# ReallyNecessarySherbert/VoxelHex

Hardware: AMD Instinct MI355X
Metric: primary Mrays/s at 3840×2160 on 1024³ brick tree; achieved HBM GB/s % (higher is better)
Workload: dtype f32; 1 GPU; primary rays 3840x2160, 1024^3 procedural scene S (lattice+cube), brick_dim 4, glass camera; workload_key=primary 3840x2160 S1 1024^3 bd4 ranks1, tree_size=1024, brick_dim=4, width=3840, height=2160, scene=1, parallelism=single GPU, tree_nodes=187246, tree_bricks=11796480

## Files before the change

### voxelhex_amd/csrc/ctx.hpp

```cpp
#pragma once
#include <hip/hip_runtime.h>

#include <condition_variable>
#include <cstdint>
#include <memory>
#include <mutex>
#include <string>
#include <vector>

#include "../../include/vhx.h"

struct DevBuf {
    void *ptr = nullptr;
    uint64_t bytes = 0;
};

struct TreeStore {
    int device = 0;
    bool uploaded = false;
    vhx_tree_desc desc{};
    DevBuf raw[7];
    DevBuf hdr, brick_occ;
    DevBuf child_rec;
    bool child_rec_stale = false;
// ... 67 lines not shown
    DevBuf upd;
    DevBuf query;
    hipStream_t upd_stream = nullptr;
    struct BuildScratch {
        DevBuf occ, rank, first, part, table, ctl, grid, simp;
    } build;
    struct EditScratch {
        DevBuf oldn, aft, need, rank, nmask, first, ctl;
    } edit;
    struct CompactScratch {
        DevBuf new_of, old_of, nmask, nrank, bmask, bfirst, bnew, bsrc, ctl;
    } compact;
    bool prepass = false, in_prepass = false;
    bool shadow_on = false;
    float shadow_light[3] = {0.f, 0.f, 0.f};
    bool keep_ev0 = false;
    uint32_t shadow_budget = 0;
    bool tail_on = false;
    uint32_t tail_min = 512, tail_cap = 4096, tail_rpw = 4, tail_prio = 0;
    DevBuf tail_list[2], tail_mask;
    uint32_t tail_cur = 0, tail_w = 0, tail_h = 0;
    bool tail_valid = false;
    uint32_t *tail_rec = nullptr;
    hipStream_t tail_stream = nullptr;
    hipEvent_t tail_fork = nullptr, tail_join = nullptr;
    float prepass_margin = 0.0f;
    DevBuf prepass_depth;
    struct Sched {
        uint32_t budgets[VHX_MAX_BUDGETS];
        uint32_t npass;
        uint32_t sparse[VHX_MAX_BUDGETS];
        uint32_t queue_waves_per_cu;
        uint32_t qorder;
        uint32_t qsort;
        uint32_t queue_waves0_per_cu;
        uint32_t shadow_budgets[VHX_MAX_BUDGETS];
        uint32_t shadow_npass;
    };
    bool adaptive = true;
    Sched sched_busy = {{32u, 128u, 768u}, 4u, {12u}, 3u, VHX_QORDER_BUSY, VHX_QSORT_BUSY, 4u, {24u, 72u, 216u, 648u}, 5u};
    Sched sched_idle = {{64u}, 2u, {0u}, 8u, VHX_QORDER_IDLE, VHX_QSORT_IDLE, 32u, {64u}, 2u};
    int last_sched = -1;
    uint32_t budgets[VHX_MAX_BUDGETS] = {32u, 128u, 768u};
    uint32_t npass = 4;
    uint32_t rpw[VHX_MAX_BUDGETS + 1] = {64u, 64u, 64u, 64u, 64u, 64u, 64u};
    uint32_t tw = 1024;
    uint32_t scan_multi = 8;
    bool p0lists = true;
    bool resume = true;
    bool qstate = false;
    bool tile_lists = true;
    bool frame_interleave = true;
    bool skyblocks = true;
    DevBuf sky;
    uint32_t save_from = 0;
    uint32_t xcd_group = 16;
    uint32_t qblock = 256;
    uint32_t queue_blocks = 2048;
    uint32_t queue_waves = 1024;
    uint32_t cus = 256;
    uint32_t queue_waves0 = 8192;
    uint32_t queue_waves0_force = 0;
    uint32_t queue_waves_mid = 0;
    uint32_t qxcd = 16;
    bool qxcd_all = false;
    uint32_t qorder = VHX_QORDER_BUSY;
    uint32_t last_fb_w = 0, last_fb_h = 0;
    uint32_t sparse[VHX_MAX_BUDGETS] = {12u};
    uint32_t qsort = 0;
    int qsort_force = -1;
    uint32_t qsort_passes = 0xFEu;
    uint32_t qsort_blocks = 2048u;
};

#define VHX_HIP(ctx, call)                                                                                         \
    do {                                                                                                           \
        hipError_t e_ = (call);                                                                                    \
        if (e_ != hipSuccess) {                                                                                    \
            (ctx)->err = std::string(#call) + ": " + hipGetErrorString(e_);                                        \
            return VHX_E_HIP;                                                                                      \
        }                                                                                                          \
    } while (0)

#define VHX_STREAM(ctx)                                                                                            \
    do {                                                                                                           \
        if (!(ctx)->stream) {                                                                                      \
            if (!(ctx)->own_stream) VHX_HIP(ctx, hipStreamCreateWithFlags(&(ctx)->own_stream, hipStreamNonBlocking)); \
            (ctx)->stream = (ctx)->own_stream;                                                                     \
        }                                                                                                          \
    } while (0)

static inline int fail(vhx_ctx *ctx, int code, const char *msg) {
    if (ctx) ctx->err = msg;
    return code;
}
static inline int fail(vhx_ctx *ctx, int code, const std::string &msg) { return fail(ctx, code, msg.c_str()); }

namespace vhx {
int ensure(vhx_ctx *c, DevBuf &b, uint64_t bytes);
uint64_t elem_size(int id);
uint64_t elem_count(const vhx_tree_desc &d, int id);
int alloc_tree(vhx_ctx *c, const vhx_tree_desc *t);
int grow_tree(vhx_ctx *c, const vhx_tree_desc *t);
int finish_upload(vhx_ctx *c);
struct FreshTree {
    DevBuf raw[7], hdr, brick_occ, child_rec;
};
// ... 53 lines not shown
```

### voxelhex_amd/csrc/vhx_ctx.hip

```cpp
#include <hip/hip_runtime.h>

#include <algorithm>
#include <cmath>
#include <cstdio>
#include <cstdlib>
#include <cstring>
#include <string>
#include <vector>

#include "../../include/vhx.h"
#include "ctx.hpp"

using namespace vhx;

__global__ void __launch_bounds__(256) k_untile_planes(const uint32_t *__restrict__ gathered, uint32_t planes,
                                                       uint32_t ranks, uint32_t tiles_per_rank, uint32_t T,
                                                       uint32_t tiles_x, uint32_t ntiles, uint32_t width,
                                                       uint32_t height, uint32_t *__restrict__ fb0,
                                                       uint32_t *__restrict__ fb1) {
    const uint64_t i = (uint64_t)blockIdx.x * blockDim.x + threadIdx.x;
    const uint64_t per_plane = (uint64_t)tiles_per_rank * T * T, per_rank = per_plane * planes;
    if (i >= per_rank * ranks) return;
    const uint32_t r = (uint32_t)(i / per_rank);
    const uint64_t w = i - (uint64_t)r * per_rank;
// ... 128 lines not shown
    if (hipGetDeviceCount(&n) != hipSuccess || n == 0) return VHX_E_NO_DEVICE;
    if (hip_device < 0 || hip_device >= n) return VHX_E_INVALID_ARG;
    vhx_ctx *c = new vhx_ctx();
    c->device = hip_device;
    c->tree = std::make_shared<TreeStore>();
    c->tree->device = hip_device;
    register_user(c);
    auto bail = [&](const char *what, hipError_t e) {
        fprintf(stderr, "vhx_create: %s: %s\n", what, hipGetErrorString(e));
        delete c;
        return VHX_E_HIP;
    };
    hipError_t e;
    if ((e = hipSetDevice(hip_device)) != hipSuccess) return bail("hipSetDevice", e);
    {
        hipDeviceProp_t prop;
        if (hipGetDeviceProperties(&prop, hip_device) == hipSuccess && prop.multiProcessorCount > 0) {
            c->cus = (uint32_t)prop.multiProcessorCount;
            c->queue_blocks = c->cus * 8u;
            c->queue_waves = c->sched_busy.queue_waves_per_cu * c->cus;
        }
    }
    if ((e = hipEventCreate(&c->ev0)) != hipSuccess) return bail("hipEventCreate", e);
    if ((e = hipEventCreate(&c->ev1)) != hipSuccess) return bail("hipEventCreate", e);
    *out = c;
    return VHX_OK;
}

int vhx_create_shared(const vhx_ctx *owner, vhx_ctx **out) {
    if (!owner || !out) return VHX_E_INVALID_ARG;
    *out = nullptr;
    vhx_ctx *c = nullptr;
    int rc = vhx_create(owner->device, &c);
    if (rc) return rc;
    c->tree = owner->tree;
    register_user(c);
    c->shared = true;
    copy_sched(c, owner);
    *out = c;
    return VHX_OK;
}

void vhx_destroy(vhx_ctx *c) {
    if (!c) return;
    (void)hipSetDevice(c->device);
    if (c->stream) (void)hipStreamSynchronize(c->stream);
    unregister_user(c);
    c->tree.reset();
    if (c->use_ev) (void)hipEventDestroy(c->use_ev);
    for (DevBuf *b : {&c->scratch, &c->rays, &c->queue[0], &c->queue[1], &c->qctl, &c->tmp, &c->counts, &c->offsets,
                      &c->flags, &c->qargs, &c->state, &c->stateq, &c->upd, &c->prepass_depth, &c->batch_args, &c->scan_part,
                      &c->shadow_args, &c->tail_list[0], &c->tail_list[1], &c->tail_mask, &c->build.occ, &c->build.rank,
                      &c->build.first, &c->build.part, &c->build.table, &c->build.ctl, &c->build.grid,
                      &c->build.simp, &c->sky, &c->query, &c->edit.oldn, &c->edit.aft, &c->edit.need,
                      &c->edit.rank, &c->edit.nmask, &c->edit.first, &c->edit.ctl, &c->compact.new_of,
                      &c->compact.old_of, &c->compact.nmask, &c->compact.nrank, &c->compact.bmask,
                      &c->compact.bfirst, &c->compact.bnew, &c->compact.bsrc, &c->compact.ctl})
        if (b->ptr) (void)hipFree(b->ptr);
    if (c->tail_stream) {
        (void)hipStreamSynchronize(c->tail_stream);
        (void)hipStreamDestroy(c->tail_stream);
    }
    if (c->tail_fork) (void)hipEventDestroy(c->tail_fork);
    if (c->tail_join) (void)hipEventDestroy(c->tail_join);
    std::vector<vhx_ctx::Pinned *> pins = {&c->pinned[0], &c->pinned[1]};
    for (auto &P : c->batch_pinned) pins.push_back(&P);
    for (auto &P : c->shadow_pinned) pins.push_back(&P);
    for (auto *P : pins) {
        if (P->ptr) (void)hipHostFree(P->ptr);
        if (P->done) (void)hipEventDestroy(P->done);
    }
    if (c->ev0) (void)hipEventDestroy(c->ev0);
    if (c->ev1) (void)hipEventDestroy(c->ev1);
    if (c->own_stream) (void)hipStreamDestroy(c->own_stream);
    delete c;
}

static bool parse_u32_list(const std::string &v, uint32_t *out, uint32_t cap, uint32_t &n) {
    n = 0;
    const char *q = v.c_str();
    if (!*q) return true;
    for (;;) {
        char *end = nullptr;
        const unsigned long x = strtoul(q, &end, 10);
        if (end == q || n >= cap || x > 0xFFFFFFFFul) return false;
        out[n++] = (uint32_t)x;
        if (*end == '\0') return true;
        if (*end != ',') return false;
        q = end + 1;
    }
}
static bool parse_u32(const std::string &v, uint32_t &out) {
    uint32_t n = 0, x[1];
    if (!parse_u32_list(v, x, 1, n) || n != 1) return false;
    out = x[0];
    return true;
}
static int apply_tuning(vhx_ctx *c, const std::string &key, const std::string &val) {
    uint32_t x = 0, n = 0, l[VHX_MAX_BUDGETS + 1];
    auto bad = [&]() { return fail(c, VHX_E_INVALID_ARG, ("vhx_set_tuning: bad value for " + key).c_str()); };
    if (key == "budgets") {
        if (!parse_u32_list(val, l, VHX_MAX_BUDGETS, n)) return bad();
        if (n == 1 && l[0] == 0) n = 0;
        return vhx_set_pass_budgets(c, l, n);
    } else if (key == "adaptive") {
        if (!parse_u32(val, x) || x > 1) return bad();
        return vhx_set_adaptive_schedule(c, (int)x);
// ... 304 lines not shown
```

### voxelhex_amd/csrc/vhx_device.hip

```cpp
#include <hip/hip_runtime.h>

#include <algorithm>
#include <cmath>
#include <cstdio>
#include <cstdlib>
#include <cstring>
#include <string>
#include <vector>

#include "../../include/vhx.h"
#include "trace.hpp"
#define VHX_SKY_FN __host__ __device__
#include "skyblock.hpp"
static_assert(VHX_RAY_GLASS == 1u, "skyblock.hpp spells the glass model's number out (it includes no header)");

using namespace vhx;

#include "ctx.hpp"

struct CamD {
    uint32_t model, width, height;
    float ox, oy, oz;
    float blx, bly, blz, rx, ry, rz, ux, uy, uz, pw, ph;
    float m[16];
};

struct OutD {
    uint32_t *value, *cell, *voxel, *rgba, *bytes;
    float *impact, *normal, *depth;
    uint32_t *shadowed;
};

__device__ __forceinline__ uint32_t shade(const DevTree &t, const HitOut &h) {
    if (!h.hit) return 128u | (128u << 8) | (128u << 16) | (255u << 24);
    const uint32_t ci = h.value & 0xFFFFu;
    if (ci == 0xFFFFu || ci >= t.color_count) return 255u << 24;
    const uint32_t c = t.color[ci];
    const F3d L = vnorm(mk(0.0f, -1.0f, 1.0f));
    const float dot = (h.nx * L.x + h.ny * L.y) + h.nz * L.z;
    const float s = 1.0f - (dot / 2.0f + 0.5f);
    const uint32_t r = ras_u8((float)(c & 0xFFu) * s), g = ras_u8((float)((c >> 8) & 0xFFu) * s),
                   b = ras_u8((float)((c >> 16) & 0xFFu) * s);
    return r | (g << 8) | (b << 16) | (255u << 24);
}

__device__ __forceinline__ void store(const DevTree &t, const OutD &o, uint64_t i, F3d org, const HitOut &h) {
    if (o.value) o.value[i] = h.hit ? h.value : VHX_EMPTY;
    if (o.cell) o.cell[i] = h.hit ? h.cell : VHX_EMPTY;
    if (o.voxel) {
        o.voxel[3 * i] = h.hit ? h.vx : VHX_EMPTY;
        o.voxel[3 * i + 1] = h.hit ? h.vy : VHX_EMPTY;
        o.voxel[3 * i + 2] = h.hit ? h.vz : VHX_EMPTY;
    }
    if (o.impact) {
        o.impact[3 * i] = h.hit ? h.ix : 0.0f;
        o.impact[3 * i + 1] = h.hit ? h.iy : 0.0f;
        o.impact[3 * i + 2] = h.hit ? h.iz : 0.0f;
    }
    if (o.normal) {
        o.normal[3 * i] = h.hit ? h.nx : 0.0f;
        o.normal[3 * i + 1] = h.hit ? h.ny : 0.0f;
        o.normal[3 * i + 2] = h.hit ? h.nz : 0.0f;
    }
    if (o.depth) o.depth[i] = h.hit ? vlen(vsub(mk(h.ix, h.iy, h.iz), org)) : __builtin_huge_valf();
    if (o.rgba) o.rgba[i] = shade(t, h);
    if (o.bytes) o.bytes[i] = h.bytes;
}

__device__ __forceinline__ void primary_ray(const CamD &c, uint32_t px, uint32_t py, F3d &o, F3d &d) {
    const uint32_t x = px, y = c.height - 1u - py;
    o = mk(c.ox, c.oy, c.oz);
    if (c.model == VHX_RAY_GLASS) {
        const F3d gp = vadd(vadd(mk(c.blx, c.bly, c.blz), vmul(vmul(mk(c.rx, c.ry, c.rz), (float)x), c.pw)),
                            vmul(vmul(mk(c.ux, c.uy, c.uz), (float)y), c.ph));
        d = vnorm(vsub(gp, o));
    } else {
        const float nx = ((float)x + 0.5f) / (float)c.width * 2.0f - 1.0f;
        const float ny = ((float)y + 0.5f) / (float)c.height * 2.0f - 1.0f;
        float nr[4], fr[4];
#pragma unroll
        for (int k = 0; k < 4; ++k) {
            nr[k] = ((c.m[k] * nx + c.m[4 + k] * ny) + c.m[8 + k] * -1.0f) + c.m[12 + k] * 1.0f;
            fr[k] = ((c.m[k] * nx + c.m[4 + k] * ny) + c.m[8 + k] * 1.0f) + c.m[12 + k] * 1.0f;
        }
        const F3d np = mk(nr[0] / nr[3], nr[1] / nr[3], nr[2] / nr[3]);
        const F3d fp = mk(fr[0] / fr[3], fr[1] / fr[3], fr[2] / fr[3]);
        const F3d dd = vsub(fp, np);
        const float rcp = 1.0f / __builtin_sqrtf((dd.x * dd.x + dd.y * dd.y) + dd.z * dd.z);
        d = vmul(dd, rcp);
    }
}

__device__ __forceinline__ bool glass_clear_miss(const CamD &c, uint32_t px, uint32_t py, float tsize) {
    if (c.model != VHX_RAY_GLASS) return false;
    const uint32_t x = px, y = c.height - 1u - py;
    const F3d o = mk(c.ox, c.oy, c.oz);
    const F3d gp = vadd(vadd(mk(c.blx, c.bly, c.blz), vmul(vmul(mk(c.rx, c.ry, c.rz), (float)x), c.pw)),
                        vmul(vmul(mk(c.ux, c.uy, c.uz), (float)y), c.ph));
    const F3d v = vsub(gp, o);
    const float vk[3] = {v.x, v.y, v.z}, ok[3] = {o.x, o.y, o.z};
    float tmin = -__builtin_huge_valf(), tmax = __builtin_huge_valf();
    bool safe = true;
#pragma unroll
    for (int k = 0; k < 3; ++k) {
        safe = safe && __builtin_fabsf(vk[k]) > 1e-20f;
        const float r = __builtin_amdgcn_rcpf(vk[k]);
        const float t1 = (0.0f - ok[k]) * r, t2 = (tsize - ok[k]) * r;
        tmin = __builtin_fmaxf(tmin, __builtin_fminf(t1, t2));
        tmax = __builtin_fminf(tmax, __builtin_fmaxf(t1, t2));
    }
    if (!safe || !__builtin_isfinite(tmin) || !__builtin_isfinite(tmax)) return false;
    const float m = 1e-5f * __builtin_fmaxf(__builtin_fabsf(tmin), __builtin_fabsf(tmax));
    return tmax < -m || tmin - tmax > m;
}

__global__ void __launch_bounds__(256) k_classify_sky(const CamD *__restrict__ cams, uint32_t nfr, uint32_t blocks_x,
                                                      uint32_t blocks_y, uint32_t tree_size,
                                                      uint8_t *__restrict__ mask) {
    const uint32_t nb = blocks_x * blocks_y;
    const uint32_t i = blockIdx.x * 256u + threadIdx.x;
    if (i >= nfr * nb) return;
    const uint32_t f = i / nb, b = i - f * nb, by = b / blocks_x, bx = b - by * blocks_x;
    const CamD &c = cams[f];
    const SkyCam s{c.model, c.width, c.height, {c.ox, c.oy, c.oz}, {c.blx, c.bly, c.blz}, {c.rx, c.ry, c.rz},
                   {c.ux, c.uy, c.uz}, c.pw, c.ph};
    const uint32_t x1 = min(bx * 16u + 15u, c.width - 1u), y1 = min(by * 16u + 15u, c.height - 1u);
    mask[i] = block_is_sky(s, tree_size, bx * 16u, by * 16u, x1, y1) ? 1 : 0;
}

struct PassQ {
    uint32_t budget;
    uint32_t rpw;
    uint32_t tw;
    uint32_t resume;
    uint32_t *tmp;
    uint32_t *counts;
    uint8_t *flags;
    uint4 *state;
    const uint4 *sin;
    uint32_t qmode;
    uint32_t xcd_group;
    uint32_t qxcd;
    uint32_t sparse;
    uint32_t *zero;
    float lx, ly, lz;
    uint32_t sbud;
    const uint32_t *skip;
    uint32_t *tail_out;
    uint32_t tail_min, tail_cap;
    uint32_t finter;
};

__device__ __forceinline__ void tail_record(uint32_t *list, uint32_t cap, uint32_t idx) {
    const uint32_t k = atomicAdd(list, 1u);
    if (k < cap) list[64u + k] = idx;
}

__device__ __forceinline__ uint32_t pass_rpw(uint32_t rpw, uint32_t tw, uint32_t n) {
    if (rpw) return rpw;
    const uint32_t k = (n + tw - 1) / tw;
    return k < 1u ? 1u : (k > 64u ? 64u : k);
}

__device__ __forceinline__ void block_append(bool push, uint32_t idx, uint32_t *tmp, uint32_t *counts,
                                             uint32_t pos) {
    __shared__ uint32_t s_cnt[4];
    const uint32_t wave = threadIdx.x >> 6, lane = threadIdx.x & 63u;
    const uint64_t m = __ballot(push);
    if (lane == 0) s_cnt[wave] = (uint32_t)__popcll(m);
    __syncthreads();
    uint32_t before = 0;
    for (uint32_t w = 0; w < wave; ++w) before += s_cnt[w];
    if (push) tmp[(uint64_t)pos * 256u + before + (uint32_t)__popcll(m & ((1ull << lane) - 1ull))] = idx;
    if (threadIdx.x == 0) counts[pos] = s_cnt[0] + s_cnt[1] + s_cnt[2] + s_cnt[3];
}

#define SCAN_THREADS 256u
__device__ __forceinline__ uint32_t wave_incl_scan(uint32_t v, uint32_t lane) {
    for (uint32_t d = 1; d < 64; d <<= 1) {
        const uint32_t x = __shfl_up(v, d);
// ... 511 lines not shown
struct UDiv {
    uint32_t m, sh;
};
static UDiv udiv_of(uint32_t d) {
    if (d == 0u) return UDiv{0u, 0u};
    uint32_t l = 0;
    while ((1ull << l) < d) ++l;
    return UDiv{(uint32_t)(((1ull << (31u + l)) + d - 1u) / d), 31u + l};
}
__device__ __forceinline__ uint32_t udiv(uint32_t n, const UDiv &d) { return (uint32_t)(((uint64_t)n * d.m) >> d.sh); }

struct BatchGrid {
    uint32_t nfr;
    uint32_t xfull;
    uint32_t xshift;
    UDiv xg;
    UDiv split;
    UDiv ltx, bx;
    UDiv bpt, bpx, tiles_x;
    uint32_t sbx, sby, W, H;
};
static BatchGrid batch_grid(uint32_t nblocks, uint32_t nfr, uint32_t nblocks_frame, uint32_t blocks_x, const PassQ &q,
                            const ListOrder &lo, const TileB &tb) {
    BatchGrid g{};
    const uint32_t G = q.xcd_group;
    g.nfr = nfr;
    g.xfull = G && 8ull * G <= nblocks ? (uint32_t)(nblocks / (8ull * G) * (8ull * G)) : 0u;
    g.xshift = ~0u;
    if (G && (G & (G - 1u)) == 0u)
        for (g.xshift = 0; (1u << g.xshift) < G;) ++g.xshift;
    g.xg = udiv_of(G);
    g.split = udiv_of(q.finter ? nfr : nblocks_frame);
    g.ltx = udiv_of(lo.tx);
    g.bx = udiv_of(blocks_x);
    g.bpt = udiv_of(tb.bpt);
    g.bpx = udiv_of(tb.bpx);
    g.tiles_x = udiv_of(tb.tiles_x);
    return g;
}
__device__ __forceinline__ uint32_t xcd_block(uint32_t bid, uint32_t G, const BatchGrid &g) {
    if (bid >= g.xfull) return bid;
    const uint32_t x = bid & 7u, k = bid >> 3;
    if (g.xshift != ~0u) return ((((k >> g.xshift) << 3) + x) << g.xshift) + (k & (G - 1u));
    const uint32_t kq = udiv(k, g.xg);
    return (kq * 8u + x) * G + (k - kq * G);
}
__device__ __forceinline__ void list_block(const ListOrder &lo, const UDiv &ltx, uint32_t b, uint32_t &bx,
                                           uint32_t &by) {
    const uint32_t tb = b >> (2u * lo.tbl), m = b & ((1u << (2u * lo.tbl)) - 1u);
    const uint32_t ty = udiv(tb, ltx);
    bx = ((tb - ty * lo.tx) << lo.tbl) + compact_bits(m);
    by = (ty << lo.tbl) + compact_bits(m >> 1);
}

template <int BD, bool FUSE = false>
__global__ void __launch_bounds__(256) VHX_BATCH_ATTR k_trace_primary_batch(DevTree t, const CamD *__restrict__ cams,
                                                             const OutD *__restrict__ outs, uint32_t nblocks_frame,
                                                             uint32_t blocks_x, uint32_t npix, PassQ q, BatchGrid bg,
                                                             ListOrder lo = ListOrder{}, TileB tb = TileB{},
                                                             const uint32_t *__restrict__ starts = nullptr,
                                                             const uint32_t *__restrict__ sky = nullptr) {
    __shared__ uint64_t occ_tab[OCC_TAB_WORDS];
    zero_ctl(q.zero);
    const uint32_t bid = __builtin_amdgcn_readfirstlane(xcd_block(blockIdx.x, q.xcd_group, bg));
    const uint32_t bq = udiv(bid, bg.split);
    const uint32_t f = __builtin_amdgcn_readfirstlane(q.finter ? bid - bq * bg.nfr : bq);
    const uint32_t sb = __builtin_amdgcn_readfirstlane(q.finter ? bq : bid - bq * nblocks_frame);
    const uint32_t wave = __builtin_amdgcn_readfirstlane(threadIdx.x >> 6), lane = threadIdx.x & 63u;
    uint32_t px = 0, py = 0, local;
    if (!tb.T) {
        uint32_t bx, by;
        if (lo.tx) {
            list_block(lo, bg.ltx, sb, bx, by);
            px = bx * 16u + (wave & 1u) * 8u + compact_bits(lane);
            py = by * 16u + (wave >> 1) * 8u + compact_bits(lane >> 1);
        } else {
            by = udiv(sb, bg.bx);
            bx = sb - by * blocks_x;
            px = bx * 16u + (wave & 1u) * 8u + (lane & 7u);
            py = by * 16u + (wave >> 1) * 8u + (lane >> 3);
        }
        if (!FUSE && sky) {
            const bool inside = bx < bg.sbx && by < bg.sby;
            const uint32_t mi = inside ? f * (bg.sbx * bg.sby) + by * bg.sbx + bx : 0u;
            const uint32_t word = sky[mi >> 2];
            const OutD out = outs[f];
            asm volatile("" ::"s"(word), "s"(out.value), "s"(out.cell), "s"(out.voxel), "s"(out.rgba), "s"(out.impact),
                         "s"(out.normal), "s"(out.depth));
            if (!inside || ((word >> ((mi & 3u) * 8u)) & 1u) != 0u) {
                local = py * bg.W + px;
                if (px < bg.W && py < bg.H) {
                    HitOut h;
                    h.hit = false;
                    h.bytes = 0;
                    store(t, out, local, mk(0.0f, 0.0f, 0.0f), h);
                    if (q.flags) q.flags[(uint64_t)f * npix + local] = 0;
                }
                if ((lo.tx || lo.tl) && q.tmp) wave_append(false, 0u, q.tmp, q.counts, bid * 4u + wave);
                return;
            }
        }
    }
    fill_occ_tab(occ_tab);
    __syncthreads();
    const CamD cam = cams[f];
    bool valid, entry;
    if (tb.T) {
        const uint32_t j = __builtin_amdgcn_readfirstlane(udiv(sb, bg.bpt)), sbb = sb - j * tb.bpt;
        const uint32_t sby = udiv(sbb, bg.bpx);
        const uint32_t lx = (sbb - sby * tb.bpx) * 16u + (wave & 1u) * 8u + (lane & 7u);
        const uint32_t ly = sby * 16u + (wave >> 1) * 8u + (lane >> 3);
        const uint32_t tile = __builtin_amdgcn_readfirstlane(starts[f] + j * tb.stride);
        const uint32_t tyy = udiv(tile, bg.tiles_x);
        px = (tile - tyy * tb.tiles_x) * tb.T + lx;
        py = tyy * tb.T + ly;
        entry = lx < tb.T && ly < tb.T;
        valid = entry && tile < tb.ntiles && px < cam.width && py < cam.height;
        local = (j * tb.T + ly) * tb.T + lx;
    } else {
        valid = entry = px < cam.width && py < cam.height;
        local = py * cam.width + px;
    }
    const uint64_t idx = (uint64_t)f * npix + local;
    bool done = true;
    uint32_t tag = 0u;
    if (valid) {
        F3d o, d;
        HitOut h;
        h.bytes = 0;
        if (glass_clear_miss(cam, px, py, (float)t.size)) {
            o = mk(cam.ox, cam.oy, cam.oz);
            h.hit = false;
            h.iters = 0;
        } else {
            primary_ray(cam, px, py, o, d);
            done = get_by_ray<false, BD>(t, occ_tab, o, d, h, q.budget, q.state,
                                         q.qmode ? (bid * 4u + wave) * 64u : (uint32_t)idx, false, 0.0f, q.sparse,
                                         nullptr, 0, q.qmode != 0);
        }
        if (done) {
            const OutD out = outs[f];
            store(t, out, local, o, h);
            if (FUSE && !fused_shadow<BD>(t, occ_tab, q, out, local, h, (uint32_t)idx)) {
                done = false;
                tag = VHX_QSHADOW;
            }
        }
    }
    if (q.flags && entry) q.flags[idx] = done ? 0 : 1;
    if ((lo.tx || lo.tl) && q.tmp) wave_append(!done, (uint32_t)idx | tag, q.tmp, q.counts, bid * 4u + wave);
}

template <bool COUNT, int BD, bool MIP = false>
__global__ void __launch_bounds__(256) k_trace_rays(DevTree t, const float *__restrict__ rays, uint64_t n, OutD out,
                                                    PassQ q) {
    __shared__ uint64_t occ_tab[OCC_TAB_WORDS];
    fill_occ_tab(occ_tab);
    __syncthreads();
    const uint64_t i = (uint64_t)blockIdx.x * blockDim.x + threadIdx.x;
    bool done = true;
    if (i < n) {
        const F3d o = mk(rays[6 * i], rays[6 * i + 1], rays[6 * i + 2]);
        const F3d d = mk(rays[6 * i + 3], rays[6 * i + 4], rays[6 * i + 5]);
        HitOut h;
        h.bytes = 0;
        done = get_by_ray<COUNT, BD, false, MIP>(t, occ_tab, o, d, h, q.budget, q.state, (uint32_t)i);
        if (done)
            store(t, out, i, o, h);
        else if (COUNT && q.state)
            out.bytes[i] = h.bytes;
    }
    if (q.tmp) block_append(!done, (uint32_t)i, q.tmp, q.counts, blockIdx.x);
}


#if VHX_CHAIN
#define VHX_CHAIN_WORDS 64u
template <int BD>
__global__ void __launch_bounds__(64) k_chain(DevTree t, CamD cam, const uint32_t *__restrict__ pix, uint32_t n,
                                              unsigned long long *__restrict__ out) {
    __shared__ uint64_t occ_tab[OCC_TAB_WORDS];
    fill_occ_tab(occ_tab);
    __syncthreads();
    if (threadIdx.x != 0 || blockIdx.x >= n) return;
    const uint32_t idx = pix[blockIdx.x], py = idx / cam.width, px = idx - py * cam.width;
    F3d o, d;
    primary_ray(cam, px, py, o, d);
    HitOut h;
    h.bytes = 0;
    h.chain = ChainAcc{};
    const unsigned long long t0 = chain_stamp();
    get_by_ray<false, BD>(t, occ_tab, o, d, h, VHX_MAX_ITERS);
    const unsigned long long t1 = chain_stamp();
    unsigned long long *w = out + (uint64_t)blockIdx.x * VHX_CHAIN_WORDS;
    const unsigned long long v[11] = {t1 - t0,        h.chain.load,   h.chain.probe, h.chain.move,
                                      h.chain.adv,    h.chain.other,  h.chain.nload, h.chain.nprobe,
                                      h.chain.nadv,   h.iters,        h.hit ? h.value : VHX_EMPTY};
    for (uint32_t k = 0; k < 11u; ++k) w[k] = v[k];
    for (uint32_t k = 0; k < VHX_CHAIN_HIST; ++k) w[16 + k] = h.chain.hist[k];
}
#endif

__device__ __forceinline__ void store_shadow(const OutD &o, uint64_t i, const HitOut &h) {
// ... 428 lines not shown
    return rc;
}

static int put_qargs(vhx_ctx *c, const CamD &cam, const RaySrc &src, const OutD &o, QueueArgs *&qa) {
    const uint32_t slot = src.kind == 3u || src.kind == 5u ? 1u : 0u;
    qa = (QueueArgs *)c->qargs.ptr + slot;
    QueueArgs a;
    std::memset(&a, 0, sizeof(a));
    a.cam = cam;
    a.src = src;
    a.out = o;
    const uint8_t *ab = (const uint8_t *)&a;
    if (c->qargs_host_ptr[slot] != c->qargs.ptr || c->qargs_host[slot].size() != sizeof(a) ||
        std::memcmp(c->qargs_host[slot].data(), ab, sizeof(a)) != 0) {
        k_put_queue_args<<<1, 64, 0, c->stream>>>(a, qa);
        VHX_HIP(c, hipGetLastError());
        c->qargs_host[slot].assign(ab, ab + sizeof(a));
        c->qargs_host_ptr[slot] = c->qargs.ptr;
    }
    return VHX_OK;
}

enum { P0_LISTS = 0, P0_FLAGS = 1, P0_ORDERED = 2 };

template <bool HITS>
static int compact_flags(vhx_ctx *c, const void *src, uint64_t npos, const FlagOrder &ord, uint32_t *total,
                         uint32_t *out, uint32_t *clear = nullptr, uint64_t nclear = 0) {
    const unsigned nb = (unsigned)((npos + 1023) / 1024);
    if ((uint64_t)nb * 4 > c->counts.bytes || (uint64_t)nb * 4 > c->offsets.bytes) {
        const int rc = ensure_lists(c, nb);
        if (rc) return rc;
    }
    uint32_t *counts = (uint32_t *)c->counts.ptr, *offsets = (uint32_t *)c->offsets.ptr;
    k_count_flags<HITS><<<nb, 256, 0, c->stream>>>(src, npos, counts, (uint32_t *)c->qctl.ptr + 16, clear, ord, nclear);
    launch_scan(c, counts, nb, nullptr, 1, offsets, total, nb);
    k_emit_flags<HITS><<<nb, 256, 0, c->stream>>>(src, npos, offsets, out, ord);
    VHX_HIP(c, hipGetLastError());
    debug_passes(c, "compacted flags");
    return VHX_OK;
}

struct QueueRun {
    CamD cam{};
    RaySrc src{};
    OutD out{};
    uint32_t first = 1;
    uint32_t npass = 1;
    uint64_t nout = 0;
    uint64_t nblocks0 = 0;
    int pass0 = P0_LISTS;
    uint32_t order_w = 0, order_h = 0;
    uint32_t frames = 1;
    bool qm = false;
};

template <bool COUNT, int BD, bool MIP = false, bool FUSE = false>
static int launch_queue_passes(vhx_ctx *c, const DevTree &t, const QueueRun &r) {
    const uint32_t npass = r.npass;
    uint32_t *ctl = (uint32_t *)c->qctl.ptr, *queue0 = (uint32_t *)c->queue[0].ptr;
    int rc = VHX_OK;
    if (r.first > 0 && npass > 1) {
        if (r.pass0 == P0_FLAGS) {
            uint64_t npos = r.nout;
            const FlagOrder ord = flag_order(c->qorder, r.order_w, r.order_h, npos, r.frames);
            if ((rc = compact_flags<false>(c, c->flags.ptr, npos, ord, ctl, queue0))) return rc;
            if ((rc = sort_segments(c, 1, npass, queue0, ctl, r.nout))) return rc;
        } else if (r.pass0 == P0_ORDERED) {
            rc = compact_chunks(c, (uint32_t)(r.nblocks0 * 4), nullptr, 64, 64, queue0, ctl, r.nblocks0 * 4, r.qm);
            if (!rc) rc = sort_segments(c, 1, npass, queue0, ctl, r.nout);
        } else {
            rc = compact_chunks(c, (uint32_t)r.nblocks0, nullptr, 256, 256, queue0, ctl, r.nblocks0);
        }
    }
    QueueArgs *qa = nullptr;
    if (r.first < npass && (rc = put_qargs(c, r.cam, r.src, r.out, qa))) return rc;
    for (uint32_t p = r.first; p < npass && !rc; ++p) {
        const uint32_t *in = (const uint32_t *)c->queue[(p - 1) & 1u].ptr;
        const uint32_t *in_n = p > 0 ? ctl + (p - 1) : ctl + 7;
        const PassQ q = pass_q(c, p, npass, r.qm);
        uint32_t qwaves = p == 0 ? c->queue_waves0
                          : (p + 1 < npass && c->queue_waves_mid ? c->queue_waves_mid : c->queue_waves);
        if (r.frames > 1 && p > 0) qwaves = (uint32_t)std::min<uint64_t>((uint64_t)qwaves * r.frames, 20ull * c->cus);
        const unsigned qgrid = (qwaves * 64u + c->qblock - 1) / c->qblock;
        uint32_t *grab = ctl + 16u + QCTL_PASS_WORDS * p;
        if constexpr (!FUSE && !MIP) {
            if (q.qmode)
                k_trace_queue<COUNT, BD, MIP, FUSE, true><<<qgrid, c->qblock, 0, c->stream>>>(t, qa, in, in_n, grab, q);
            else
                k_trace_queue<COUNT, BD, MIP, FUSE><<<qgrid, c->qblock, 0, c->stream>>>(t, qa, in, in_n, grab, q);
        } else {
            k_trace_queue<COUNT, BD, MIP, FUSE><<<qgrid, c->qblock, 0, c->stream>>>(t, qa, in, in_n, grab, q);
        }
        debug_passes(c, "queue pass");
        if (p + 1 < npass) {
            rc = compact_chunks(c, 0, in_n, q.rpw, q.rpw, (uint32_t *)c->queue[p & 1u].ptr, ctl + p,
                                q.rpw ? (r.nout + q.rpw - 1) / q.rpw : r.nout, r.qm);
            if (!rc) rc = sort_segments(c, p + 1, npass, (uint32_t *)c->queue[p & 1u].ptr, ctl + p, r.nout);
        }
    }
    return rc;
}

template <bool C, bool M, bool F, bool S>
struct VarTag {
    static constexpr bool COUNT = C, MIP = M, FUSE = F, FAST = S;
};
template <class Fn>
static bool dispatch_variant(uint32_t bd, bool mip, bool count, bool fuse, bool fast, Fn &&f) {
    return dispatch_bd(bd, [&](auto b) {
        if (mip) f(b, VarTag<false, true, false, false>{});
        else if (count) f(b, VarTag<true, false, false, false>{});
        else if (fuse) f(b, VarTag<false, false, true, false>{});
        else if (fast) f(b, VarTag<false, false, false, true>{});
        else f(b, VarTag<false, false, false, false>{});
    });
}

struct TraceCall {
    vhx_ctx *c;
    const bool nested;
    int rc;
// ... 356 lines not shown
        if (outs[k].bytes)
            return fail(c, VHX_E_INVALID_ARG, std::string(fn) + ": byte counting is a vhx_trace_primary option");
        if (c->shadow_on && (!outs[k].value || !outs[k].impact || !outs[k].normal || !outs[k].shadowed))
            return fail(c, VHX_E_INVALID_ARG, std::string(fn) + " with a shadow light: value, impact, normal and "
                                              "shadowed outputs needed");
    }
    const uint32_t tiles_x = T ? (W + T - 1) / T : 0u, ntiles = T ? tiles_x * ((H + T - 1) / T) : 0u;
    const uint32_t bpx = T ? (T + 15) / 16 : 0u, bpt = bpx * bpx;
    auto set_tiles = [&](uint32_t k) -> uint64_t {
        return starts[k] >= ntiles ? 0ull : (uint64_t)(ntiles - starts[k] + stride - 1) / stride;
    };
    uint64_t max_tiles = 0;
    if (T)
        for (uint32_t k = 0; k < n; ++k) max_tiles = std::max(max_tiles, set_tiles(k));
    if (T && max_tiles == 0) return VHX_OK;
    const uint64_t npix = T ? max_tiles * T * T : (uint64_t)W * H, nout = npix * n;
    {
        std::vector<MemRange> written;
        for (uint32_t k = 0; k < n; ++k) {
            const vhx_hits &o = outs[k];
            const uint64_t ent = T ? set_tiles(k) * T * T : npix;
            const void *f[7] = {o.value, o.cell, o.rgba, o.depth, o.voxel, o.impact, o.normal};
            const uint64_t w[7] = {1, 1, 1, 1, 3, 3, 3};
            for (int j = 0; j < 7; ++j) written.push_back({f[j], ent * 4 * w[j]});
        }
        if (ranges_meet(written, {}))
            return fail(c, VHX_E_INVALID_ARG, std::string(fn) + ": output arrays overlap each other");
    }
    const uint32_t bx = (W + 15) / 16, by = (H + 15) / 16;
    const uint64_t nbf = T ? max_tiles * bpt : (uint64_t)bx * by, nblocks = nbf * n;
    if (nout > 0x7FFFFFFFull || nblocks > 0x7FFFFFFFull)
        return fail(c, VHX_E_INVALID_ARG, std::string(fn) + ": more than 2^31 rays in one batch");
    TraceCall tr(c);
    int rc = tr.rc;
    if (rc) return rc;
    DevTree t;
    if ((rc = tr.tree(t))) return rc;
    if (t.mips) return fail(c, VHX_E_INVALID_ARG, std::string(fn) + ": not available with node MIPs");
    const uint64_t cam_bytes = ((uint64_t)n * sizeof(CamD) + 255) & ~255ull;
    const uint64_t out_bytes = ((uint64_t)n * sizeof(OutD) + 255) & ~255ull;
    const uint64_t args_bytes = cam_bytes + out_bytes + (T ? (uint64_t)n * 4 : 0ull);
    vhx_ctx::Pinned *P = nullptr;
    if ((rc = stage_acquire(c, c->batch_pinned, c->batch_next, c->batch_args, args_bytes, P))) return rc;
    CamD *hc = (CamD *)P->ptr;
    OutD *ho = (OutD *)((uint8_t *)P->ptr + cam_bytes);
    for (uint32_t k = 0; k < n; ++k) {
        hc[k] = cam_of(&cams[k]);
        ho[k] = OutD{outs[k].value, outs[k].cell,   outs[k].voxel, outs[k].rgba,
                     nullptr,       outs[k].impact, outs[k].normal, outs[k].depth, outs[k].shadowed};
    }
    if (T) std::memcpy((uint8_t *)P->ptr + cam_bytes + out_bytes, starts, (size_t)n * 4);
    uint32_t npass = 1;
    if ((rc = prepare_passes(c, nout, nblocks, npass, false, n > 1))) return rc;
    const bool sky = c->skyblocks && !T;
    if (sky && (rc = ensure(c, c->sky, ((uint64_t)bx * by * n + 3) & ~3ull))) return rc;
    if ((rc = tr.start()) || (rc = stage_commit(c, *P, c->batch_args, args_bytes))) return rc;
    const CamD *dcams = (const CamD *)c->batch_args.ptr;
    const OutD *douts = (const OutD *)((const uint8_t *)c->batch_args.ptr + cam_bytes);
    const uint32_t *dstarts = T ? (const uint32_t *)((const uint8_t *)c->batch_args.ptr + cam_bytes + out_bytes) : nullptr;
    const TileB tb{T, tiles_x, ntiles, stride, bpx, bpt};
    Pass0Plan p0;
    if ((rc = plan_pass0(c, npass, !T, T != 0, W, H, nbf, n, c->shadow_on, false, p0))) return rc;
    QueueRun run;
    run.src.kind = 4u;
    run.src.cams = dcams;
    run.src.outs = douts;
    run.src.npix = (uint32_t)npix;
    run.src.T = T;
    run.src.tiles_x = tiles_x;
    run.src.tile_stride = stride;
    run.src.starts = dstarts;
    run.npass = npass;
    run.nout = nout;
    run.nblocks0 = p0.nbf * n;
    run.pass0 = p0.p0();
    run.order_w = T ? 0u : W;
    run.order_h = H;
    run.frames = n;
    run.qm = p0.qm;
    const PassQ q0 = pass0_q(c, npass, run.pass0, p0.qm);
    BatchGrid bg = batch_grid((uint32_t)run.nblocks0, n, (uint32_t)p0.nbf, bx, q0, p0.lo, tb);
    const uint32_t *dsky = nullptr;
    if (sky && !p0.fuse) {
        const uint32_t nsky = bx * by * n;
        k_classify_sky<<<(nsky + 255u) / 256u, 256, 0, c->stream>>>(dcams, n, bx, by, t.size, (uint8_t *)c->sky.ptr);
        dsky = (const uint32_t *)c->sky.ptr;
        bg.sbx = bx;
        bg.sby = by;
        bg.W = W;
        bg.H = H;
    }
    int qrc = VHX_OK;
    const bool bd_ok = dispatch_variant(c->tree->desc.brick_dim, false, false, p0.fuse, false, [&](auto bd_tag, auto v) {
        constexpr int BD = decltype(bd_tag)::value;
        constexpr bool FUSE = decltype(v)::FUSE;
        k_trace_primary_batch<BD, FUSE><<<(unsigned)run.nblocks0, 256, 0, c->stream>>>(
            t, dcams, douts, (uint32_t)p0.nbf, bx, (uint32_t)npix, q0, bg, p0.lo, tb, dstarts, dsky);
        qrc = launch_queue_passes<false, BD, false, FUSE>(c, t, run);
    });
    if (!bd_ok) return fail(c, VHX_E_INVALID_ARG, "unsupported brick_dim");
    if ((rc = tr.end(qrc))) return rc;
    c->last_fb_w = T ? 0u : W;
    c->last_fb_h = T ? 0u : H;
    if (c->shadow_on && !p0.fuse) {
        c->keep_ev0 = true;
        for (uint32_t k = 0; k < n && !rc; ++k) {
            const uint64_t ent = T ? set_tiles(k) * T * T : npix;
            if (ent)
                rc = vhx_trace_shadows(c, c->shadow_light, ent, outs[k].value, outs[k].impact, outs[k].normal,
                                       outs[k].shadowed, outs[k].rgba, nullptr);
        }
        c->keep_ev0 = false;
    }
    return rc;
}

int vhx_trace_primary_batch(vhx_ctx *c, const vhx_camera *cams, uint32_t n, const vhx_hits *outs) {
    return trace_batch(c, cams, n, outs, 0, nullptr, 1, "vhx_trace_primary_batch");
}

int vhx_trace_tiles_batch(vhx_ctx *c, const vhx_camera *cams, uint32_t n, uint32_t tile_size, const uint32_t *tile_starts,
                          uint32_t tile_stride, const vhx_hits *outs) {
    if (tile_size == 0) return c ? fail(c, VHX_E_INVALID_ARG, "vhx_trace_tiles_batch: tile_size 0") : VHX_E_INVALID_ARG;
    return trace_batch(c, cams, n, outs, tile_size, tile_starts, tile_stride, "vhx_trace_tiles_batch");
}


int vhx_tail_info(vhx_ctx *c, uint32_t *listed, uint32_t *width, uint32_t *height) {
    if (!c) return VHX_E_INVALID_ARG;
    uint32_t n = 0;
    if (c->tail_on && c->tail_valid && c->tail_list[c->tail_cur].ptr) {
        VHX_HIP(c, hipSetDevice(c->device));
        VHX_STREAM(c);
        VHX_HIP(c, hipMemcpyAsync(&n, c->tail_list[c->tail_cur].ptr, 4, hipMemcpyDeviceToHost, c->stream));
        VHX_HIP(c, hipStreamSynchronize(c->stream));
        n = std::min(n, c->tail_cap);
    }
    if (listed) *listed = n;
    if (width) *width = c->tail_valid ? c->tail_w : 0u;
    if (height) *height = c->tail_valid ? c->tail_h : 0u;
    return VHX_OK;
}

int vhx_chain_profile(vhx_ctx *c, const vhx_camera *cam, const uint32_t *pixels, uint32_t n, uint64_t *out) {
    if (!c || !cam || (n && (!pixels || !out))) return VHX_E_INVALID_ARG;
#if VHX_CHAIN
    if (!c->tree->uploaded) return fail(c, VHX_E_STATE, "vhx_chain_profile before vhx_upload_tree");
    if (n == 0) return VHX_OK;
    for (uint32_t k = 0; k < n; ++k)
        if (pixels[k] >= (uint64_t)cam->width * cam->height) return fail(c, VHX_E_INVALID_ARG, "vhx_chain_profile: pixel outside the frame");
// ... 212 lines not shown
```

Before: 19090 Mrays/s.

## Replace per-block sky mask with compacted tree/sky worklist for primary batch

Sky classification now yields a compacted worklist via ballot, a scan, and an emit kernel. Tree blocks are launched first and sky blocks after. Sky blocks use a single wave that writes miss values with vectorised 16-byte stores instead of full store() calls, and they no longer append empty entries to the wave queue. Pass-0 compaction reads the tree-only count from the worklist. This adds two extra kernels and a scan, and it only applies when the ordered/listed pass-0 path is active.

```diff
diff --git a/voxelhex_amd/csrc/ctx.hpp b/voxelhex_amd/csrc/ctx.hpp
--- a/voxelhex_amd/csrc/ctx.hpp
+++ b/voxelhex_amd/csrc/ctx.hpp
@@ -143,7 +143,7 @@
     bool tile_lists = true;
     bool frame_interleave = true;
     bool skyblocks = true;
-    DevBuf sky;
+    DevBuf work;
     uint32_t save_from = 0;
     uint32_t xcd_group = 16;
     uint32_t qblock = 256;
diff --git a/voxelhex_amd/csrc/vhx_ctx.hip b/voxelhex_amd/csrc/vhx_ctx.hip
--- a/voxelhex_amd/csrc/vhx_ctx.hip
+++ b/voxelhex_amd/csrc/vhx_ctx.hip
@@ -204,7 +204,7 @@
                       &c->flags, &c->qargs, &c->state, &c->stateq, &c->upd, &c->prepass_depth, &c->batch_args, &c->scan_part,
                       &c->shadow_args, &c->tail_list[0], &c->tail_list[1], &c->tail_mask, &c->build.occ, &c->build.rank,
                       &c->build.first, &c->build.part, &c->build.table, &c->build.ctl, &c->build.grid,
-                      &c->build.simp, &c->sky, &c->query, &c->edit.oldn, &c->edit.aft, &c->edit.need,
+                      &c->build.simp, &c->work, &c->query, &c->edit.oldn, &c->edit.aft, &c->edit.need,
                       &c->edit.rank, &c->edit.nmask, &c->edit.first, &c->edit.ctl, &c->compact.new_of,
                       &c->compact.old_of, &c->compact.nmask, &c->compact.nrank, &c->compact.bmask,
                       &c->compact.bfirst, &c->compact.bnew, &c->compact.bsrc, &c->compact.ctl})
diff --git a/voxelhex_amd/csrc/vhx_device.hip b/voxelhex_amd/csrc/vhx_device.hip
--- a/voxelhex_amd/csrc/vhx_device.hip
+++ b/voxelhex_amd/csrc/vhx_device.hip
@@ -31,8 +31,9 @@
     uint32_t *shadowed;
 };
 
+#define VHX_MISS_RGBA (128u | (128u << 8) | (128u << 16) | (255u << 24))
 __device__ __forceinline__ uint32_t shade(const DevTree &t, const HitOut &h) {
-    if (!h.hit) return 128u | (128u << 8) | (128u << 16) | (255u << 24);
+    if (!h.hit) return VHX_MISS_RGBA;
     const uint32_t ci = h.value & 0xFFFFu;
     if (ci == 0xFFFFu || ci >= t.color_count) return 255u << 24;
     const uint32_t c = t.color[ci];
@@ -65,6 +66,34 @@
     if (o.depth) o.depth[i] = h.hit ? vlen(vsub(mk(h.ix, h.iy, h.iz), org)) : __builtin_huge_valf();
     if (o.rgba) o.rgba[i] = shade(t, h);
     if (o.bytes) o.bytes[i] = h.bytes;
+}
+
+template <int WORDS, class T, class T4>
+__device__ __forceinline__ void fill_miss(T *plane, uint64_t i, uint32_t npx, T v) {
+    if (!plane) return;
+    T *a = plane + WORDS * i;
+    if (npx == 4u && ((uintptr_t)a & 15u) == 0u) {
+        T4 v4;
+        v4.x = v4.y = v4.z = v4.w = v;
+#pragma unroll
+        for (int k = 0; k < WORDS; ++k) ((T4 *)a)[k] = v4;
+    } else {
+        for (uint32_t k = 0; k < WORDS * npx; ++k) a[k] = v;
+    }
+}
+__device__ __forceinline__ void store_miss_block(const OutD &o, uint32_t bx, uint32_t by, uint32_t W, uint32_t H) {
+    const uint32_t lane = threadIdx.x & 63u;
+    const uint32_t x = bx * 16u + (lane & 3u) * 4u, y = by * 16u + (lane >> 2);
+    if (x >= W || y >= H) return;
+    const uint64_t i = (uint64_t)y * W + x;
+    const uint32_t npx = W - x < 4u ? W - x : 4u;
+    fill_miss<1, uint32_t, uint4>(o.value, i, npx, VHX_EMPTY);
+    fill_miss<1, uint32_t, uint4>(o.cell, i, npx, VHX_EMPTY);
+    fill_miss<3, uint32_t, uint4>(o.voxel, i, npx, VHX_EMPTY);
+    fill_miss<3, float, float4>(o.impact, i, npx, 0.0f);
+    fill_miss<3, float, float4>(o.normal, i, npx, 0.0f);
+    fill_miss<1, float, float4>(o.depth, i, npx, __builtin_huge_valf());
+    fill_miss<1, uint32_t, uint4>(o.rgba, i, npx, VHX_MISS_RGBA);
 }
 
 __device__ __forceinline__ void primary_ray(const CamD &c, uint32_t px, uint32_t py, F3d &o, F3d &d) {
@@ -112,20 +141,6 @@
     if (!safe || !__builtin_isfinite(tmin) || !__builtin_isfinite(tmax)) return false;
     const float m = 1e-5f * __builtin_fmaxf(__builtin_fabsf(tmin), __builtin_fabsf(tmax));
     return tmax < -m || tmin - tmax > m;
-}
-
-__global__ void __launch_bounds__(256) k_classify_sky(const CamD *__restrict__ cams, uint32_t nfr, uint32_t blocks_x,
-                                                      uint32_t blocks_y, uint32_t tree_size,
-                                                      uint8_t *__restrict__ mask) {
-    const uint32_t nb = blocks_x * blocks_y;
-    const uint32_t i = blockIdx.x * 256u + threadIdx.x;
-    if (i >= nfr * nb) return;
-    const uint32_t f = i / nb, b = i - f * nb, by = b / blocks_x, bx = b - by * blocks_x;
-    const CamD &c = cams[f];
-    const SkyCam s{c.model, c.width, c.height, {c.ox, c.oy, c.oz}, {c.blx, c.bly, c.blz}, {c.rx, c.ry, c.rz},
-                   {c.ux, c.uy, c.uz}, c.pw, c.ph};
-    const uint32_t x1 = min(bx * 16u + 15u, c.width - 1u), y1 = min(by * 16u + 15u, c.height - 1u);
-    mask[i] = block_is_sky(s, tree_size, bx * 16u, by * 16u, x1, y1) ? 1 : 0;
 }
 
 struct PassQ {
@@ -743,6 +758,76 @@
     bx = ((tb - ty * lo.tx) << lo.tbl) + compact_bits(m);
     by = (ty << lo.tbl) + compact_bits(m >> 1);
 }
+__device__ __forceinline__ uint32_t xcd_block_n(uint32_t bid, uint32_t n, uint32_t G, const BatchGrid &g) {
+    if (G == 0u) return bid;
+    uint32_t full;
+    if (g.xshift != ~0u) full = g.xshift >= 29u ? 0u : (n >> (g.xshift + 3u)) << (g.xshift + 3u);
+    else full = udiv(n >> 3, g.xg) * 8u * G;
+    if (bid >= full) return bid;
+    const uint32_t x = bid & 7u, k = bid >> 3;
+    if (g.xshift != ~0u) return ((((k >> g.xshift) << 3) + x) << g.xshift) + (k & (G - 1u));
+    const uint32_t kq = udiv(k, g.xg);
+    return (kq * 8u + x) * G + (k - kq * G);
+}
+__device__ __forceinline__ void batch_split(uint32_t bid, uint32_t finter, uint32_t nblocks_frame, const BatchGrid &g,
+                                            uint32_t &f, uint32_t &sb) {
+    const uint32_t bq = udiv(bid, g.split);
+    f = finter ? bid - bq * g.nfr : bq;
+    sb = finter ? bq : bid - bq * nblocks_frame;
+}
+
+#define WORK_HDR 64u
+__global__ void __launch_bounds__(256) k_classify_blocks(const CamD *__restrict__ cams, BatchGrid bg, ListOrder lo,
+                                                         uint32_t nblocks_frame, uint32_t finter, uint32_t nblocks,
+                                                         uint32_t tree_size, uint64_t *__restrict__ masks,
+                                                         uint32_t *__restrict__ counts) {
+    __shared__ uint32_t s_cnt[8];
+    const uint32_t p = blockIdx.x * 256u + threadIdx.x;
+    bool tree = false, sky = false;
+    if (p < nblocks) {
+        uint32_t f, sb, bx, by;
+        batch_split(p, finter, nblocks_frame, bg, f, sb);
+        list_block(lo, bg.ltx, sb, bx, by);
+        if (bx < bg.sbx && by < bg.sby) {
+            const CamD &c = cams[f];
+            const SkyCam s{c.model, c.width, c.height, {c.ox, c.oy, c.oz}, {c.blx, c.bly, c.blz}, {c.rx, c.ry, c.rz},
+                           {c.ux, c.uy, c.uz}, c.pw, c.ph};
+            const uint32_t x1 = min(bx * 16u + 15u, c.width - 1u), y1 = min(by * 16u + 15u, c.height - 1u);
+            sky = block_is_sky(s, tree_size, bx * 16u, by * 16u, x1, y1);
+            tree = !sky;
+        }
+    }
+    const uint64_t mt = __ballot(tree), ms = __ballot(sky);
+    const uint32_t w = p >> 6, wave = threadIdx.x >> 6;
+    if ((threadIdx.x & 63u) == 0u) {
+        masks[2u * w] = mt;
+        masks[2u * w + 1u] = ms;
+        s_cnt[wave] = (uint32_t)__popcll(mt);
+        s_cnt[4u + wave] = (uint32_t)__popcll(ms);
+    }
+    __syncthreads();
+    if (threadIdx.x == 0u) {
+        counts[blockIdx.x] = s_cnt[0] + s_cnt[1] + s_cnt[2] + s_cnt[3];
+        counts[gridDim.x + blockIdx.x] = s_cnt[4] + s_cnt[5] + s_cnt[6] + s_cnt[7];
+    }
+}
+__global__ void __launch_bounds__(256) k_emit_worklist(const uint64_t *__restrict__ masks,
+                                                       const uint32_t *__restrict__ offsets,
+                                                       uint32_t *__restrict__ work) {
+    const uint32_t p = blockIdx.x * 256u + threadIdx.x, w = p >> 6, lane = threadIdx.x & 63u;
+    if (p == 0u) {
+        work[0] = offsets[gridDim.x];
+        work[2] = offsets[gridDim.x] * 256u;
+    }
+    const uint64_t mt = masks[2u * w], ms = masks[2u * w + 1u], below = (1ull << lane) - 1ull;
+    uint32_t ot = offsets[blockIdx.x], os = offsets[gridDim.x + blockIdx.x];
+    for (uint32_t v = blockIdx.x * 4u; v < w; ++v) {
+        ot += (uint32_t)__popcll(masks[2u * v]);
+        os += (uint32_t)__popcll(masks[2u * v + 1u]);
+    }
+    if ((mt >> lane) & 1ull) work[WORK_HDR + ot + (uint32_t)__popcll(mt & below)] = p;
+    if ((ms >> lane) & 1ull) work[WORK_HDR + os + (uint32_t)__popcll(ms & below)] = p;
+}
 
 template <int BD, bool FUSE = false>
 __global__ void __launch_bounds__(256) VHX_BATCH_ATTR k_trace_primary_batch(DevTree t, const CamD *__restrict__ cams,
@@ -750,14 +835,34 @@
                                                              uint32_t blocks_x, uint32_t npix, PassQ q, BatchGrid bg,
                                                              ListOrder lo = ListOrder{}, TileB tb = TileB{},
                                                              const uint32_t *__restrict__ starts = nullptr,
-                                                             const uint32_t *__restrict__ sky = nullptr) {
+                                                             const uint32_t *__restrict__ work = nullptr) {
     __shared__ uint64_t occ_tab[OCC_TAB_WORDS];
     zero_ctl(q.zero);
-    const uint32_t bid = __builtin_amdgcn_readfirstlane(xcd_block(blockIdx.x, q.xcd_group, bg));
-    const uint32_t bq = udiv(bid, bg.split);
-    const uint32_t f = __builtin_amdgcn_readfirstlane(q.finter ? bid - bq * bg.nfr : bq);
-    const uint32_t sb = __builtin_amdgcn_readfirstlane(q.finter ? bq : bid - bq * nblocks_frame);
     const uint32_t wave = __builtin_amdgcn_readfirstlane(threadIdx.x >> 6), lane = threadIdx.x & 63u;
+    uint32_t bid, pos;
+    if (!FUSE && work) {
+        const uint32_t ntree = work[0], nall = work[1];
+        if (blockIdx.x >= nall) return;
+        if (blockIdx.x >= ntree) {
+            if (wave != 0u) return;
+            uint32_t f, sb, bx, by;
+            batch_split(__builtin_amdgcn_readfirstlane(work[WORK_HDR + blockIdx.x]), q.finter, nblocks_frame, bg, f, sb);
+            list_block(lo, bg.ltx, sb, bx, by);
+            const OutD out = outs[f];
+            asm volatile("" ::"s"(out.value), "s"(out.cell), "s"(out.voxel), "s"(out.rgba), "s"(out.impact),
+                         "s"(out.normal), "s"(out.depth));
+            store_miss_block(out, bx, by, bg.W, bg.H);
+            return;
+        }
+        pos = __builtin_amdgcn_readfirstlane(xcd_block_n(blockIdx.x, ntree, q.xcd_group, bg));
+        bid = __builtin_amdgcn_readfirstlane(work[WORK_HDR + pos]);
+    } else {
+        pos = bid = __builtin_amdgcn_readfirstlane(xcd_block(blockIdx.x, q.xcd_group, bg));
+    }
+    uint32_t f, sb;
+    batch_split(bid, q.finter, nblocks_frame, bg, f, sb);
+    f = __builtin_amdgcn_readfirstlane(f);
+    sb = __builtin_amdgcn_readfirstlane(sb);
     uint32_t px = 0, py = 0, local;
     if (!tb.T) {
         uint32_t bx, by;
@@ -770,26 +875,6 @@
             bx = sb - by * blocks_x;
             px = bx * 16u + (wave & 1u) * 8u + (lane & 7u);
             py = by * 16u + (wave >> 1) * 8u + (lane >> 3);
-        }
-        if (!FUSE && sky) {
-            const bool inside = bx < bg.sbx && by < bg.sby;
-            const uint32_t mi = inside ? f * (bg.sbx * bg.sby) + by * bg.sbx + bx : 0u;
-            const uint32_t word = sky[mi >> 2];
-            const OutD out = outs[f];
-            asm volatile("" ::"s"(word), "s"(out.value), "s"(out.cell), "s"(out.voxel), "s"(out.rgba), "s"(out.impact),
-                         "s"(out.normal), "s"(out.depth));
-            if (!inside || ((word >> ((mi & 3u) * 8u)) & 1u) != 0u) {
-                local = py * bg.W + px;
-                if (px < bg.W && py < bg.H) {
-                    HitOut h;
-                    h.hit = false;
-                    h.bytes = 0;
-                    store(t, out, local, mk(0.0f, 0.0f, 0.0f), h);
-                    if (q.flags) q.flags[(uint64_t)f * npix + local] = 0;
-                }
-                if ((lo.tx || lo.tl) && q.tmp) wave_append(false, 0u, q.tmp, q.counts, bid * 4u + wave);
-                return;
-            }
         }
     }
     fill_occ_tab(occ_tab);
@@ -826,7 +911,7 @@
         } else {
             primary_ray(cam, px, py, o, d);
             done = get_by_ray<false, BD>(t, occ_tab, o, d, h, q.budget, q.state,
-                                         q.qmode ? (bid * 4u + wave) * 64u : (uint32_t)idx, false, 0.0f, q.sparse,
+                                         q.qmode ? (pos * 4u + wave) * 64u : (uint32_t)idx, false, 0.0f, q.sparse,
                                          nullptr, 0, q.qmode != 0);
         }
         if (done) {
@@ -839,7 +924,7 @@
         }
     }
     if (q.flags && entry) q.flags[idx] = done ? 0 : 1;
-    if ((lo.tx || lo.tl) && q.tmp) wave_append(!done, (uint32_t)idx | tag, q.tmp, q.counts, bid * 4u + wave);
+    if ((lo.tx || lo.tl) && q.tmp) wave_append(!done, (uint32_t)idx | tag, q.tmp, q.counts, pos * 4u + wave);
 }
 
 template <bool COUNT, int BD, bool MIP = false>
@@ -1374,6 +1459,7 @@
     uint32_t order_w = 0, order_h = 0;
     uint32_t frames = 1;
     bool qm = false;
+    const uint32_t *n0 = nullptr;
 };
 
 template <bool COUNT, int BD, bool MIP = false, bool FUSE = false>
@@ -1388,7 +1474,7 @@
             if ((rc = compact_flags<false>(c, c->flags.ptr, npos, ord, ctl, queue0))) return rc;
             if ((rc = sort_segments(c, 1, npass, queue0, ctl, r.nout))) return rc;
         } else if (r.pass0 == P0_ORDERED) {
-            rc = compact_chunks(c, (uint32_t)(r.nblocks0 * 4), nullptr, 64, 64, queue0, ctl, r.nblocks0 * 4, r.qm);
+            rc = compact_chunks(c, (uint32_t)(r.nblocks0 * 4), r.n0, 64, 64, queue0, ctl, r.nblocks0 * 4, r.qm);
             if (!rc) rc = sort_segments(c, 1, npass, queue0, ctl, r.nout);
         } else {
             rc = compact_chunks(c, (uint32_t)r.nblocks0, nullptr, 256, 256, queue0, ctl, r.nblocks0);
@@ -1851,8 +1937,6 @@
     if (T) std::memcpy((uint8_t *)P->ptr + cam_bytes + out_bytes, starts, (size_t)n * 4);
     uint32_t npass = 1;
     if ((rc = prepare_passes(c, nout, nblocks, npass, false, n > 1))) return rc;
-    const bool sky = c->skyblocks && !T;
-    if (sky && (rc = ensure(c, c->sky, ((uint64_t)bx * by * n + 3) & ~3ull))) return rc;
     if ((rc = tr.start()) || (rc = stage_commit(c, *P, c->batch_args, args_bytes))) return rc;
     const CamD *dcams = (const CamD *)c->batch_args.ptr;
     const OutD *douts = (const OutD *)((const uint8_t *)c->batch_args.ptr + cam_bytes);
@@ -1879,22 +1963,31 @@
     run.qm = p0.qm;
     const PassQ q0 = pass0_q(c, npass, run.pass0, p0.qm);
     BatchGrid bg = batch_grid((uint32_t)run.nblocks0, n, (uint32_t)p0.nbf, bx, q0, p0.lo, tb);
-    const uint32_t *dsky = nullptr;
-    if (sky && !p0.fuse) {
-        const uint32_t nsky = bx * by * n;
-        k_classify_sky<<<(nsky + 255u) / 256u, 256, 0, c->stream>>>(dcams, n, bx, by, t.size, (uint8_t *)c->sky.ptr);
-        dsky = (const uint32_t *)c->sky.ptr;
+    const uint32_t *dwork = nullptr;
+    if (c->skyblocks && !T && p0.listed && p0.lo.tx && !p0.fuse && ((uint64_t)bx * by * n + 1) * 256 <= 0xFFFFFFFFull) {
+        const uint32_t nb0 = (uint32_t)run.nblocks0, ng = (nb0 + 255u) / 256u;
+        const uint64_t ent_words = (WORK_HDR + (uint64_t)nb0 + 1) & ~1ull;
+        if ((rc = ensure(c, c->work, (ent_words + 20ull * ng) * 4))) return rc;
+        uint32_t *work = (uint32_t *)c->work.ptr;
+        uint64_t *masks = (uint64_t *)(work + ent_words);
+        uint32_t *wcounts = work + ent_words + 16ull * ng, *woffsets = wcounts + 2ull * ng;
         bg.sbx = bx;
         bg.sby = by;
         bg.W = W;
         bg.H = H;
+        k_classify_blocks<<<ng, 256, 0, c->stream>>>(dcams, bg, p0.lo, (uint32_t)p0.nbf, q0.finter, nb0, t.size, masks,
+                                                      wcounts);
+        launch_scan(c, wcounts, 2u * ng, nullptr, 1, woffsets, work + 1, 2ull * ng);
+        k_emit_worklist<<<ng, 256, 0, c->stream>>>(masks, woffsets, work);
+        dwork = work;
+        run.n0 = work + 2;
     }
     int qrc = VHX_OK;
     const bool bd_ok = dispatch_variant(c->tree->desc.brick_dim, false, false, p0.fuse, false, [&](auto bd_tag, auto v) {
         constexpr int BD = decltype(bd_tag)::value;
         constexpr bool FUSE = decltype(v)::FUSE;
         k_trace_primary_batch<BD, FUSE><<<(unsigned)run.nblocks0, 256, 0, c->stream>>>(
-            t, dcams, douts, (uint32_t)p0.nbf, bx, (uint32_t)npix, q0, bg, p0.lo, tb, dstarts, dsky);
+            t, dcams, douts, (uint32_t)p0.nbf, bx, (uint32_t)npix, q0, bg, p0.lo, tb, dstarts, dwork);
         qrc = launch_queue_passes<false, BD, false, FUSE>(c, t, run);
     });
     if (!bd_ok) return fail(c, VHX_E_INVALID_ARG, "unsupported brick_dim");
```

Result: faster. 19660 Mrays/s, median of 6 (+3.0%).
